# mindspore-lab/mindpose

Hardware: AMD Instinct MI355X
Metric: images/sec at 256x192, HRNet-W32 top-down inference (backbone+head+decode) (higher is better)
Workload: dtype f32; 1 GPU; configs[2]: HRNet-W32 256x192 inference, 1xMI355X per rank, multi-branch conv + fuse layers on fp32 MFMA, HRNetHead, arg-max+shift decode; per_gpu_batch=128, global_batch=128, image=256x192, heatmap=64x48x17, execution_lanes=4

## Files before the change

include/mindpose_hip.h:

```cpp
#ifndef MINDPOSE_HIP_H
#define MINDPOSE_HIP_H

#include <stddef.h>
#include <stdint.h>

#ifdef __cplusplus
extern "C" {
#endif

typedef void* mp_stream_t;

#define MP_OK 0
#define MP_ERR_NULL (-1)
#define MP_ERR_SHAPE (-2)
#define MP_ERR_UNSUPPORTED (-3)
#define MP_ERR_HIP (-4)
#define MP_ERR_WORKSPACE (-5)

const char* mp_version(void);
const char* mp_error_string(int code);
int mp_last_hip_error(void);

#define MP_REFINE_NONE 0
#define MP_REFINE_SHIFT 1
// ... 40 lines not shown

typedef struct mp_conv_desc {
    int32_t n, cin, h, w;
    int32_t cout, kh, kw;
    int32_t stride;
    int32_t pad_top, pad_left;
    int32_t conv_h, conv_w;
    int32_t out_h, out_w;
    int32_t out_mul, out_rep, out_off_y, out_off_x;
    int32_t relu;
    int32_t flags;
} mp_conv_desc;

#define MP_CONV_SHARES_CUS 1
#define MP_CONV_PHASES4 2

size_t mp_conv_packed_weight_bytes(int cout, int cin, int kh, int kw);
int mp_conv_pack_weight(const float* w_dev, float* packed_dev, int cout, int cin, int kh, int kw,
                        int transposed, int phase_y, int phase_x, mp_stream_t stream);
int mp_conv2d_fwd(const mp_conv_desc* desc, const float* x_dev, const float* packed_w_dev,
                  const float* scale_dev, const float* shift_dev, const float* res1_dev, const float* res2_dev,
                  float* out_dev, mp_stream_t stream);

int mp_conv2d_fwd_variant(const mp_conv_desc* desc, int variant, const float* x_dev, const float* packed_w_dev,
                          const float* scale_dev, const float* shift_dev, const float* res1_dev, const float* res2_dev,
                          float* out_dev, mp_stream_t stream);

size_t mp_conv_winograd_packed_weight_bytes(int cout, int cin);
int mp_conv_winograd_pack_weight(const float* w_dev, float* packed_dev, int cout, int cin, mp_stream_t stream);
int mp_conv_winograd_supported(const mp_conv_desc* desc);
int mp_conv2d_winograd_fwd(const mp_conv_desc* desc, const float* x_dev, const float* packed_u_dev, const float* scale_dev,
                           const float* shift_dev, const float* res1_dev, const float* res2_dev, float* out_dev,
                           mp_stream_t stream);

int mp_maxpool3x3s2_same(const float* x_dev, float* out_dev, int n, int c, int h, int w, mp_stream_t stream);

int mp_fuse_upsample_sum(const float* base_dev, const float* t1_dev, int s1, const float* t2_dev, int s2,
                         const float* t3_dev, int s3, float* out_dev, int n, int c, int h, int w, int relu,
                         mp_stream_t stream);

typedef struct mp_plan mp_plan;
mp_plan* mp_plan_create(void);
void mp_plan_destroy(mp_plan* plan);
int mp_plan_add_conv(mp_plan* plan, const mp_conv_desc* desc, const float* x_dev, const float* packed_w_dev,
                     const float* scale_dev, const float* shift_dev, const float* res1_dev,
                     const float* res2_dev, float* out_dev);
int mp_plan_add_conv_variant(mp_plan* plan, const mp_conv_desc* desc, int variant, const float* x_dev,
                             const float* packed_w_dev, const float* scale_dev, const float* shift_dev,
                             const float* res1_dev, const float* res2_dev, float* out_dev);
int mp_deconv4x4s2_gemm_supported(const mp_conv_desc* phase00_desc);
int mp_deconv4x4s2_gemm_fwd(const mp_conv_desc* phase00_desc, const float* x_dev, const float* packed4_dev, const float* scale_dev,
                            const float* shift_dev, float* out_dev, mp_stream_t stream);
int mp_plan_add_deconv4x4s2_gemm(mp_plan* plan, const mp_conv_desc* phase00_desc, const float* x_dev, const float* packed4_dev,
                                 const float* scale_dev, const float* shift_dev, float* out_dev);
int mp_plan_add_conv_winograd(mp_plan* plan, const mp_conv_desc* desc, const float* x_dev, const float* packed_u_dev,
                              const float* scale_dev, const float* shift_dev, const float* res1_dev, const float* res2_dev,
                              float* out_dev);
int mp_plan_add_maxpool(mp_plan* plan, const float* x_dev, float* out_dev, int n, int c, int h, int w);
int mp_plan_add_fuse_sum(mp_plan* plan, const float* base_dev, const float* t1_dev, int s1, const float* t2_dev, int s2,
                         const float* t3_dev, int s3, float* out_dev, int n, int c, int h, int w, int relu);
int mp_plan_set_lane(mp_plan* plan, int lane);
int mp_plan_add_barrier(mp_plan* plan);
int mp_plan_size(const mp_plan* plan);
int mp_plan_run(const mp_plan* plan, mp_stream_t stream);
int mp_plan_run_range(const mp_plan* plan, int first, int count, mp_stream_t stream);
int mp_plan_entry_info(const mp_plan* plan, int index, int64_t info[12]);

size_t mp_bn_workspace_bytes(int c);
int mp_bn_train_fwd(const float* z_dev, const float* gamma_dev, const float* beta_dev, const float* res_dev, float* y_dev,
                    float* save_mean_dev, float* save_invstd_dev, float* moving_mean_dev, float* moving_var_dev, int n,
                    int c, int hw, float eps, float momentum, int relu, void* workspace_dev, size_t workspace_bytes,
                    mp_stream_t stream);
int mp_bn_train_bwd(const float* dy_dev, const float* z_dev, const float* y_dev, const float* gamma_dev,
                    const float* save_mean_dev, const float* save_invstd_dev, float* dz_dev, float* dres_dev,
                    float* dgamma_dev, float* dbeta_dev, int n, int c, int hw, int relu, void* workspace_dev,
                    size_t workspace_bytes, mp_stream_t stream);

int mp_fuse_upsample_sum_bwd(const float* dy_dev, const float* out_dev, float* dbase_dev, float* dt1_dev, int s1,
                             float* dt2_dev, int s2, float* dt3_dev, int s3, int n, int c, int h, int w, int relu,
                             mp_stream_t stream);

int mp_bn_train_bwd_acc(const float* dy_dev, const float* z_dev, const float* y_dev, const float* gamma_dev,
                        const float* save_mean_dev, const float* save_invstd_dev, float* dz_dev, float* dres_dev,
                        float* dgamma_dev, float* dbeta_dev, float* dgamma_acc_dev, float* dbeta_acc_dev, int n, int c, int hw,
                        int relu, void* workspace_dev, size_t workspace_bytes, mp_stream_t stream);

int mp_adamw_step(float* param_dev, const float* grad_dev, float* exp_avg_dev, float* exp_avg_sq_dev, size_t count,
                  float lr, float beta1, float beta2, float eps, float weight_decay, mp_stream_t stream);

int mp_adamw_step_scaled(float* param_dev, const float* grad_dev, float* exp_avg_dev, float* exp_avg_sq_dev, size_t count,
// ... 338 lines not shown
```

mindpose_amd/_lib.py:

```python
import ctypes
import os

import torch

_HERE = os.path.dirname(os.path.abspath(__file__))
LIB_PATH = os.environ.get("MINDPOSE_HIP_LIB", os.path.join(_HERE, "csrc", "libmindpose_hip.so"))

MP_REFINE_NONE, MP_REFINE_SHIFT, MP_REFINE_DARK = 0, 1, 2
MP_CONV_SHARES_CUS = 1
MP_CONV_PHASES4 = 2
MP_ERR_UNSUPPORTED = -3


def env_on(name: str, default: bool = True) -> bool:
    value = os.environ.get(name)
    return value != "0" if default else value == "1"


c_f32p = ctypes.c_void_p
c_int = ctypes.c_int
c_size_t = ctypes.c_size_t
c_i64 = ctypes.c_longlong


# ... 31 lines not shown

class BnBwdJob(ctypes.Structure):
    _fields_ = [(k, ctypes.c_void_p) for k in ("g", "z", "gamma", "save_mean", "save_invstd", "dz", "dgamma", "dbeta", "dgamma_acc",
                                                "dbeta_acc", "partials", "workspace")] + [("workspace_bytes", ctypes.c_size_t)] + \
               [(k, ctypes.c_int) for k in ("n", "c", "hw", "n_parts")]


_PROTOTYPES = {
    "mp_version": (ctypes.c_char_p, []),
    "mp_error_string": (ctypes.c_char_p, [c_int]),
    "mp_last_hip_error": (c_int, []),
    "mp_decode_topdown": (c_int, [c_f32p] * 7 + [c_int] * 7 + [ctypes.c_float, c_f32p, c_int, ctypes.c_void_p]),
    "mp_decode_topdown_debug": (c_int, [c_f32p] * 7 + [c_int] * 7 + [ctypes.c_float, c_f32p, c_int, c_f32p, ctypes.c_void_p]),
    "mp_flip_aggregate": (c_int, [c_f32p] * 4 + [c_int] * 5 + [ctypes.c_void_p]),
    "mp_flip_aggregate_decode": (c_int, [c_f32p] * 3 + [c_int] + [c_f32p] * 7 + [c_int] * 7
                                 + [ctypes.c_float, c_f32p, c_int, ctypes.c_void_p]),
    "mp_gaussian_target": (c_int, [c_f32p, c_f32p, c_int, c_f32p, c_f32p, c_f32p] + [c_int] * 4
                           + [ctypes.c_double] * 3 + [c_int, ctypes.c_void_p]),
    "mp_joints_mse_workspace_bytes": (c_size_t, [c_int, c_int]),
    "mp_joints_mse_fwd": (c_int, [c_f32p] * 5 + [c_size_t] + [c_int] * 3 + [ctypes.c_void_p]),
    "mp_joints_mse_bwd": (c_int, [c_f32p] * 5 + [c_int] * 3 + [ctypes.c_void_p]),
    "mp_joints_ohkm_workspace_bytes": (c_size_t, [c_int, c_int]),
    "mp_joints_ohkm_fwd": (c_int, [c_f32p] * 7 + [c_size_t] + [c_int] * 4 + [ctypes.c_void_p]),
    "mp_joints_ohkm_bwd": (c_int, [c_f32p] * 6 + [c_int] * 4 + [ctypes.c_void_p]),
    "mp_conv_packed_weight_bytes": (c_size_t, [c_int] * 4),
    "mp_conv_pack_weight": (c_int, [c_f32p, c_f32p] + [c_int] * 7 + [ctypes.c_void_p]),
    "mp_conv2d_fwd": (c_int, [ctypes.POINTER(ConvDesc)] + [c_f32p] * 7 + [ctypes.c_void_p]),
    "mp_conv2d_fwd_variant": (c_int, [ctypes.POINTER(ConvDesc), c_int] + [c_f32p] * 7 + [ctypes.c_void_p]),
    "mp_conv_winograd_packed_weight_bytes": (c_size_t, [c_int] * 2),
    "mp_conv_winograd_pack_weight": (c_int, [c_f32p, c_f32p, c_int, c_int, ctypes.c_void_p]),
    "mp_conv_winograd_supported": (c_int, [ctypes.POINTER(ConvDesc)]),
    "mp_conv2d_winograd_fwd": (c_int, [ctypes.POINTER(ConvDesc)] + [c_f32p] * 7 + [ctypes.c_void_p]),
    "mp_plan_add_conv_winograd": (c_int, [ctypes.c_void_p, ctypes.POINTER(ConvDesc)] + [c_f32p] * 7),
    "mp_plan_add_conv_variant": (c_int, [ctypes.c_void_p, ctypes.POINTER(ConvDesc), c_int] + [c_f32p] * 7),
    "mp_deconv4x4s2_gemm_supported": (c_int, [ctypes.POINTER(ConvDesc)]),
    "mp_deconv4x4s2_gemm_fwd": (c_int, [ctypes.POINTER(ConvDesc)] + [c_f32p] * 5 + [ctypes.c_void_p]),
    "mp_plan_add_deconv4x4s2_gemm": (c_int, [ctypes.c_void_p, ctypes.POINTER(ConvDesc)] + [c_f32p] * 5),
    "mp_maxpool3x3s2_same": (c_int, [c_f32p, c_f32p] + [c_int] * 4 + [ctypes.c_void_p]),
    "mp_fuse_upsample_sum": (c_int, [c_f32p, c_f32p, c_int, c_f32p, c_int, c_f32p, c_int, c_f32p] + [c_int] * 5 + [ctypes.c_void_p]),
    "mp_plan_add_fuse_sum": (c_int, [ctypes.c_void_p, c_f32p, c_f32p, c_int, c_f32p, c_int, c_f32p, c_int, c_f32p] + [c_int] * 5),
    "mp_plan_create": (ctypes.c_void_p, []),
    "mp_plan_destroy": (None, [ctypes.c_void_p]),
    "mp_plan_add_conv": (c_int, [ctypes.c_void_p, ctypes.POINTER(ConvDesc)] + [c_f32p] * 7),
    "mp_plan_add_maxpool": (c_int, [ctypes.c_void_p, c_f32p, c_f32p] + [c_int] * 4),
    "mp_plan_size": (c_int, [ctypes.c_void_p]),
    "mp_plan_run": (c_int, [ctypes.c_void_p, ctypes.c_void_p]),
    "mp_plan_run_range": (c_int, [ctypes.c_void_p, c_int, c_int, ctypes.c_void_p]),
    "mp_plan_entry_info": (c_int, [ctypes.c_void_p, c_int, ctypes.POINTER(ctypes.c_int64)]),
    "mp_debug_set_stamp_buffer": (c_int, [ctypes.c_void_p, c_size_t]),
    "mp_bn_workspace_bytes": (c_size_t, [c_int]),
    "mp_bn_train_fwd": (c_int, [c_f32p] * 9 + [c_int] * 3 + [ctypes.c_float, ctypes.c_float, c_int, c_f32p, c_size_t, ctypes.c_void_p]),
    "mp_bn_train_bwd": (c_int, [c_f32p] * 10 + [c_int] * 4 + [c_f32p, c_size_t, ctypes.c_void_p]),
    "mp_bn_train_bwd_acc": (c_int, [c_f32p] * 12 + [c_int] * 4 + [c_f32p, c_size_t, ctypes.c_void_p]),
    "mp_fuse_upsample_sum_bwd": (c_int, [c_f32p, c_f32p, c_f32p, c_f32p, c_int, c_f32p, c_int, c_f32p, c_int] + [c_int] * 5 + [ctypes.c_void_p]),
    "mp_conv_wgrad_workspace_bytes": (c_size_t, [ctypes.POINTER(ConvDesc)]),
    "mp_conv_wgrad": (c_int, [ctypes.POINTER(ConvDesc), c_f32p, c_f32p, c_f32p, c_int, c_f32p, c_size_t, ctypes.c_void_p]),
    "mp_adamw_step": (c_int, [c_f32p] * 4 + [c_size_t] + [ctypes.c_float] * 5 + [ctypes.c_void_p]),
    "mp_adamw_step_scaled": (c_int, [c_f32p] * 4 + [c_size_t] + [ctypes.c_float] * 6 + [c_f32p, ctypes.c_void_p]),
    "mp_grad_finite_check": (c_int, [c_f32p, c_size_t, c_f32p, ctypes.c_void_p]),
    "mp_comm_available": (c_int, []),
    "mp_comm_last_error": (c_int, []),
    "mp_comm_get_unique_id": (c_int, [ctypes.c_void_p]),
    "mp_comm_init_rank": (c_int, [ctypes.POINTER(ctypes.c_void_p), c_int, ctypes.c_void_p, c_int]),
    "mp_comm_destroy": (c_int, [ctypes.c_void_p]),
    "mp_comm_count": (c_int, [ctypes.c_void_p]),
    "mp_allreduce_grads": (c_int, [ctypes.c_void_p, c_f32p, c_size_t, c_int, ctypes.c_void_p]),
# ... 175 lines not shown
```

mindpose_amd/csrc/common.h:

```cpp
#pragma once
#include <hip/hip_runtime.h>
#include <stdint.h>
#include <stdlib.h>

#include <initializer_list>

#include "../../include/mindpose_hip.h"

namespace mp {

extern thread_local int g_last_hip_error;
extern thread_local bool g_dry_launch;

inline int check_launch() {
    hipError_t e = hipGetLastError();
    if (e != hipSuccess) {
        g_last_hip_error = (int)e;
        return MP_ERR_HIP;
    }
    return MP_OK;
}

inline hipStream_t as_stream(mp_stream_t s) { return reinterpret_cast<hipStream_t>(s); }

// ... 15 lines not shown
    if (once.need()) {
        (void)hipFuncSetAttribute(reinterpret_cast<const void*>(Kern), hipFuncAttributeMaxDynamicSharedMemorySize, 160 * 1024);
        (void)hipGetLastError();
    }
    hipLaunchKernelGGL(Kern, grid, block, lds_bytes, s, args...);
    return check_launch();
}

__device__ __forceinline__ int xcd_contiguous(int b, int nb) {
    const int q8 = nb >> 3, r8 = nb & 7, xcd = b & 7, j = b >> 3;
    return (xcd < r8 ? xcd * (q8 + 1) : r8 * (q8 + 1) + (xcd - r8) * q8) + j;
}

constexpr unsigned kOob = 0x80000000u;
__device__ __forceinline__ __amdgpu_buffer_rsrc_t make_rsrc(const void* base, size_t bytes) {
    return __builtin_amdgcn_make_buffer_rsrc(const_cast<void*>(base), 0, (int)(bytes < 0x7FFFFFF0u ? bytes : 0x7FFFFFF0u), 0x00020000);
}

inline unsigned magic_of(unsigned d) { return d <= 1 ? 0u : (unsigned)(0x100000000ULL / d) + 1u; }
__device__ __forceinline__ unsigned fastdiv(unsigned e, unsigned d, unsigned magic) { return d == 1 ? e : __umulhi(e, magic); }

inline int round_up(int v, int m) { return (v + m - 1) / m * m; }

inline bool knobs_on() {
    static const bool on = [] {
        const char* e = getenv("MINDPOSE_EXPERIMENT_KNOBS");
        return e != nullptr && atoi(e) != 0;
    }();
    return on;
}
inline const char* knob(const char* name) { return knobs_on() ? getenv(name) : nullptr; }

enum PlanKind { kConv = 0, kMaxPool = 1, kFuseSum = 2, kConvF16 = 3, kFuseSumF16 = 4, kToC8 = 5, kFromC8 = 6, kBarrier = 7, kBlockF16 = 8,
                kWinograd = 9, kPwChainF16 = 10, kStemF16 = 11, kStemF32 = 12, kPwChainF32 = 13, kConcat = 14, kColSlice = 15 };

inline void fill_info(int64_t info[12], std::initializer_list<int64_t> values) {
    int i = 0;
    for (int64_t v : values) info[i++] = v;
    for (; i < 12; ++i) info[i] = 0;
}

}
```

mindpose_amd/csrc/conv_api.hip:

```cpp
#include <stdlib.h>
#include <string.h>

#include <type_traits>
#include <variant>
#include <vector>

#include "conv_f16.h"
#include "conv_mfma.h"
#include "conv_pw.h"
#include "conv_wino.h"
#include "conv_stem.h"
#include "conv_gemm.h"
#include "conv_small.h"
#include "pwchain_f32.h"

namespace mp {

__device__ __forceinline__ float pack_source(const float* __restrict__ w, int cout, int cin, int kh, int kw, int transposed,
                                             int py, int px, int co, int ci, int t) {
    const int ty = t / kw, tx = t % kw;
    if (transposed == 0) return w[(((size_t)co * cin + ci) * kh + ty) * kw + tx];
    if (transposed == 2) {
        return w[(((size_t)ci * cout + co) * kh + (kh - 1 - ty)) * kw + (kw - 1 - tx)];
    }
    if (transposed == 3) {
        const int ky = py == 0 ? (ty == 0 ? 1 : -1) : (ty == 0 ? 2 : 0);
        const int kx = px == 0 ? (tx == 0 ? 1 : -1) : (tx == 0 ? 2 : 0);
        return (ky < 0 || kx < 0) ? 0.f : w[(((size_t)ci * cout + co) * 3 + ky) * 3 + kx];
    }
    if (transposed == 4) {
        const int my = 1 - ty, mx = 1 - tx;
        const int ky = py == 0 ? 3 - 2 * my : 2 - 2 * my;
        const int kx = px == 0 ? 3 - 2 * mx : 2 - 2 * mx;
        return w[(((size_t)co * cin + ci) * 4 + ky) * 4 + kx];
    }
    const int ky = py == 0 ? 3 - 2 * ty : 2 - 2 * ty;
    const int kx = px == 0 ? 3 - 2 * tx : 2 - 2 * tx;
    return w[(((size_t)ci * cout + co) * 4 + ky) * 4 + kx];
}

__global__ __launch_bounds__(256) void pack_weight_kernel(const float* __restrict__ w, float* __restrict__ out, int cout,
                                                          int cin, int kh, int kw, int cin_pad4, int cout_pad16,
                                                          int transposed, int py, int px) {
    const int T = kh * kw;
// ... 83 lines not shown
                     variant_light(L.variant) ? 1 : 0});
}

struct MaxPool { const float* x; float* out; int n, c, h, w; };
struct FuseSum { const float* base; const float* t[3]; int s[3]; float* out; int n, c, h, w, relu; };
struct FuseSumF16 { const void* base; const void* t[3]; int s[3]; void* out; int n, c, h, w, relu; };
struct ToC8 { const float* x; void* out; int n, c, h, w; };
struct FromC8 { const void* x; float* out; int n, c, h, w; };
struct Concat { const void* a; int ca; const void* b; int cb; void* out; int n, h, w, c8; };
struct ColSlice { const void* in; void* out; int rows, w_in, start, w_out, c8; };
struct Barrier {};

static int run(const MaxPool& r, hipStream_t s) { return mp_maxpool3x3s2_same(r.x, r.out, r.n, r.c, r.h, r.w, s); }
static int run(const FuseSum& r, hipStream_t s) {
    return mp_fuse_upsample_sum(r.base, r.t[0], r.s[0], r.t[1], r.s[1], r.t[2], r.s[2], r.out, r.n, r.c, r.h, r.w, r.relu, s);
}
static int run(const FuseSumF16& r, hipStream_t s) {
    return mp_f16_fuse_upsample_sum(r.base, r.t[0], r.s[0], r.t[1], r.s[1], r.t[2], r.s[2], r.out, r.n, r.c, r.h, r.w, r.relu, s);
}
static int run(const ToC8& r, hipStream_t s) { return mp_f16_to_c8(r.x, r.out, r.n, r.c, r.h, r.w, s); }
static int run(const FromC8& r, hipStream_t s) { return mp_f16_from_c8(r.x, r.out, r.n, r.c, r.h, r.w, s); }
static int run(const Concat& r, hipStream_t s) { return mp_concat_channels(r.a, r.ca, r.b, r.cb, r.out, r.n, r.h, r.w, r.c8, s); }
static int run(const ColSlice& r, hipStream_t s) { return mp_col_slice(r.in, r.out, r.rows, r.w_in, r.start, r.w_out, r.c8, s); }
static int run(const Barrier&, hipStream_t) { return MP_OK; }
static void describe(const MaxPool&, int64_t info[12]) { fill_info(info, {kMaxPool}); }
static void describe(const FuseSum&, int64_t info[12]) { fill_info(info, {kFuseSum}); }
static void describe(const FuseSumF16&, int64_t info[12]) { fill_info(info, {kFuseSumF16}); }
static void describe(const ToC8&, int64_t info[12]) { fill_info(info, {kToC8}); }
static void describe(const FromC8&, int64_t info[12]) { fill_info(info, {kFromC8}); }
static void describe(const Concat&, int64_t info[12]) { fill_info(info, {kConcat}); }
static void describe(const ColSlice&, int64_t info[12]) { fill_info(info, {kColSlice}); }
static void describe(const Barrier&, int64_t info[12]) { fill_info(info, {kBarrier}); }

using Record = std::variant<DirectLaunch, PwLaunch, GemmLaunch, SmallLaunch, WinoLaunch, StemF32Launch, PwChainF32Launch, ConvF16Launch,
                            BlockF16Launch, PwChainLaunch, StemF16Launch, MaxPool, FuseSum, FuseSumF16, ToC8, FromC8, Concat, ColSlice, Barrier>;
template <typename R>
constexpr bool is_f32_conv = std::is_same_v<R, DirectLaunch> || std::is_same_v<R, PwLaunch> || std::is_same_v<R, GemmLaunch> || std::is_same_v<R, SmallLaunch>;

static int run_record(const Record& rec, hipStream_t s) {
    return std::visit([s](const auto& r) { return run(r, s); }, rec);
}

static const int kLdsMax = 150 * 1024;

static int lds_budget() {
    static int v = -1;
    if (v < 0) {
        const char* e = knob("MP_CONV_LDS_KB");
        int kb = e ? atoi(e) : 0;
        v = (kb >= 16 && kb <= 150) ? kb * 1024 : 78 * 1024;
    }
    return v;
}

static int plane_pad(int raw) {
    int v = (raw + 15) / 32 * 32 + 16;
    if (v - 32 >= raw) v -= 32;
    return v;
}

static bool configure(const mp_conv_desc& d, int variant, DirectLaunch& L) {
    int CT, PT;
    variant_dims(variant, CT, PT);
    if (d.kh == 7 && variant != V_CT64_PT192 && variant != V_CT32_PT192_H) return false;
    ConvKParams& p = L.p;
    const int S = d.stride, KS = d.kh;
    p.N = d.n; p.Cin = d.cin; p.H = d.h; p.W = d.w; p.Cout = d.cout;
// ... 340 lines not shown

int mp_plan_add_maxpool(mp_plan* plan, const float* x, float* out, int n, int c, int h, int w) {
    if (!plan || !x || !out) return MP_ERR_NULL;
    if (n <= 0 || c <= 0 || h <= 0 || w <= 0) return MP_ERR_SHAPE;
    return push(plan, MaxPool{x, out, n, c, h, w});
}

int mp_plan_add_fuse_sum(mp_plan* plan, const float* base, const float* t1, int s1, const float* t2, int s2,
                         const float* t3, int s3, float* out, int n, int c, int h, int w, int relu) {
    if (!plan || !base || !t1 || !out) return MP_ERR_NULL;
    if (n <= 0 || c <= 0 || h <= 0 || w <= 0) return MP_ERR_SHAPE;
    return push(plan, FuseSum{base, {t1, t2, t3}, {s1, s2, s3}, out, n, c, h, w, relu});
}

int mp_plan_add_conv_f16(mp_plan* plan, const mp_conv_desc* desc, int variant, const void* x, const void* packed_w,
                         const float* scale, const float* shift, const void* res1, const void* res2, void* out) {
    if (!plan) return MP_ERR_NULL;
    ConvF16Launch L{};
    int rc = f16_build_launch(desc, variant, x, packed_w, scale, shift, res1, res2, out, L);
    return rc != MP_OK ? rc : push(plan, L);
}

int mp_plan_add_conv_winograd(mp_plan* plan, const mp_conv_desc* desc, const float* x, const float* packed_u, const float* scale,
                              const float* shift, const float* res1, const float* res2, float* out) {
    if (!plan) return MP_ERR_NULL;
    WinoLaunch L{};
    int rc = wino_configure(desc, L);
    if (rc != MP_OK) return rc;
    if (!x || !packed_u || !scale || !shift || !out) return MP_ERR_NULL;
    L.p.x = x; L.p.u = packed_u; L.p.scale = scale; L.p.shift = shift; L.p.res1 = res1; L.p.res2 = res2; L.p.out = out;
    return push(plan, L);
}

int mp_plan_add_basicblock_f16(mp_plan* plan, const void* x, const void* packed_w1, const float* scale1, const float* shift1,
                               const void* packed_w2, const float* scale2, const float* shift2, void* out, int n, int c, int h,
                               int w, int rows) {
    if (!plan) return MP_ERR_NULL;
    BlockF16Launch L{};
    int rc = blockf16_build(x, packed_w1, scale1, shift1, packed_w2, scale2, shift2, out, n, c, h, w, rows, L);
    return rc != MP_OK ? rc : push(plan, L);
}

int mp_plan_add_expand_reduce_f16(mp_plan* plan, const void* mid, const void* res, const void* packed_w3, const float* scale3,
                                  const float* shift3, int relu3, const void* packed_w1, const float* scale1, const float* shift1,
                                  int relu1, void* y, void* z, int n, int cm, int ce, int cr, int h, int w) {
    if (!plan) return MP_ERR_NULL;
    PwChainLaunch L{};
    int rc = pwchain_build(mid, res, packed_w3, scale3, shift3, relu3, packed_w1, scale1, shift1, relu1, y, z, n, cm, ce, cr, h, w, L);
    return rc != MP_OK ? rc : push(plan, L);
}

int mp_plan_add_expand_reduce(mp_plan* plan, const float* mid, const float* res, const float* x0, const float* packed_wd, const float* scale_d,
                              const float* shift_d, const float* packed_w3, const float* scale3, const float* shift3, const float* packed_w1,
                              const float* scale1, const float* shift1, float* y, float* z, int n, int cm, int ce, int cr, int h, int w) {
    if (!plan) return MP_ERR_NULL;
    PwChainF32Launch L{};
    int rc = pwchain32_build(mid, res, x0, packed_wd, scale_d, shift_d, packed_w3, scale3, shift3, packed_w1, scale1, shift1, y, z, n, cm, ce, cr,
                             h, w, L);
    return rc != MP_OK ? rc : push(plan, L);
}

int mp_plan_add_ds_expand_reduce_f16(mp_plan* plan, const void* mid, const void* x0, const void* packed_wd, const float* scale_d,
                                     const float* shift_d, const void* packed_w3, const float* scale3, const float* shift3, int relu3,
                                     const void* packed_w1, const float* scale1, const float* shift1, int relu1, void* y, void* z, int n,
                                     int cm, int ce, int cr, int h, int w) {
    if (!plan || !x0) return MP_ERR_NULL;
// ... 101 lines not shown
```

mindpose_amd/models/backbones/hrnet.py:

```python
import contextlib
import os
from typing import Dict, List, Tuple, Type, Union

import torch
import torch.nn as nn

from ...register import register
from .. import train_ops as T
from ..layers import BatchNorm2d, Conv2d, Plan
from .backbone import Backbone
from .utils import load_pretrained

__all__ = ["HRNet", "hrnet_w32", "hrnet_w48"]


class BasicBlock(nn.Module):

    expansion: int = 1

    def __init__(self, in_channels: int, channels: int, stride: int = 1, down_sample: nn.Module = None) -> None:
        super().__init__()
        self.conv1 = Conv2d(in_channels, channels, 3, stride=stride, padding=1)
        self.bn1 = BatchNorm2d(channels)
        self.conv2 = Conv2d(channels, channels, 3, stride=1, padding=1)
# ... 352 lines not shown
                chain = []
                for j in range(i + 1 - len(pre)):
                    cout = cur[i] if j == i - len(pre) else pre[-1]
                    chain.append(_conv_bn(pre[-1], cout, 3, stride=2, padding=1, relu=True))
                layers.append(nn.Sequential(*chain))
                flags.append(True)
        return nn.ModuleList(layers), flags

    def _make_layer(self, block, in_channels: int, out_channels: int, blocks: int, stride: int = 1) -> nn.Sequential:
        down = None
        if stride != 1 or in_channels != out_channels * block.expansion:
            down = _conv_bn(in_channels, out_channels * block.expansion, 1, stride=stride)
        layers = [block(in_channels, out_channels, stride, down_sample=down)]
        for _ in range(1, blocks):
            layers.append(block(out_channels * block.expansion, out_channels))
        return nn.Sequential(*layers)

    def _make_stage(self, cfg, num_inchannels, multi_scale_output: bool = True):
        block = self.blocks_dict[cfg["block"]]
        modules = []
        for i in range(cfg["num_modules"]):
            mso = not (not multi_scale_output and i == cfg["num_modules"] - 1)
            modules.append(HRModule(cfg["num_branches"], block, cfg["num_blocks"], num_inchannels,
                                    cfg["num_channels"], mso))
            num_inchannels = modules[-1].num_inchannels
        return nn.Sequential(*modules), num_inchannels

    def emit(self, plan: Plan, x: torch.Tensor) -> torch.Tensor:
        if plan.fuses_stem(x, self.conv1):
            x = plan.stem(x, self.conv1, self.bn1)
        else:
            x = plan.enter(x)
            x = plan.conv(x, self.conv1, self.bn1, relu=True)
        x = plan.conv(x, self.conv2, self.bn2, relu=True)
        x = emit_block_sequence(plan, list(self.layer1), x)
        ys = [x]
        for idx in (2, 3, 4):
            trans = getattr(self, f"transition{idx - 1}")
            flags = getattr(self, f"transition{idx - 1}_flags")
            cfg = getattr(self, f"stage{idx}_cfg")
            xs = []
            for i in range(cfg["num_branches"]):
                plan.set_lane(min(i, len(ys) - 1))
                if not flags[i]:
                    xs.append(ys[i])
                elif i < len(ys):
                    xs.append(_emit_conv_bn(plan, trans[i], ys[i]))
                else:
                    t = ys[-1]
                    for seq in trans[i]:
                        t = _emit_conv_bn(plan, seq, t)
                    xs.append(t)
            plan.barrier()
            for mod in getattr(self, f"stage{idx}"):
                xs = mod.emit(plan, xs)
            ys = xs
        plan.set_lane(0)
        return ys[0]

    def train_forward(self, x: torch.Tensor) -> torch.Tensor:
        if self.amp_level in ("O2", "O3") and not T._is_c8(x):
            x = T.to_c8(x)
        x = T.conv_bn_act(x, self.conv1, self.bn1, relu=True)
        x = T.conv_bn_act(x, self.conv2, self.bn2, relu=True)
        for blk in self.layer1:
            x = blk.train_forward(x)
        if x.requires_grad and x.is_cuda:
            x.register_hook(_flush_queued_weight_gradients)
        ys = [x]
        cuts = getattr(self, "_train_cut_sink", None)
        cut_at = getattr(self, "_train_cut_at", None)
        for idx in (2, 3, 4):
            if cuts is not None and (cut_at is None or idx - 2 in cut_at):
                leaves = []
                for y in ys:
                    leaf = y.detach().requires_grad_()
                    link = getattr(y, "_mp_bn_link", None)
                    if link is not None:
                        leaf._mp_bn_link = link
                    leaves.append(leaf)
                cuts.append((list(ys), leaves))
                ys = leaves
            trans = getattr(self, f"transition{idx - 1}")
            flags = getattr(self, f"transition{idx - 1}_flags")
# ... 57 lines not shown
```

mindpose_amd/models/layers.py:

```python
import ctypes
from typing import Dict, List, Optional, Tuple

import torch
import torch.nn as nn

from .. import _lib
from .act_c8 import ActC8
from .tuner import (BLOCK_ROWS, F16_VARIANTS, F32_SMALL_WIDE, F32_WINOGRAD, _autotune, autotune_on, tune_conv_variant, tuned,
                    winograd_enabled)
from .tuner import _TUNE_MIN_MACS

BN_EPS = 1e-5


class Conv2d(nn.Module):

    def __init__(self, in_channels: int, out_channels: int, kernel_size: int, stride: int = 1, padding: int = 0,
                 has_bias: bool = False) -> None:
        super().__init__()
        self.in_channels, self.out_channels = in_channels, out_channels
        self.kernel_size, self.stride, self.padding = kernel_size, stride, padding
        self.weight = nn.Parameter(torch.empty(out_channels, in_channels, kernel_size, kernel_size))
        self.bias = nn.Parameter(torch.zeros(out_channels)) if has_bias else None

# ... 232 lines not shown

    def _pack_winograd(self, weight: torch.Tensor, cout: int, cin: int) -> torch.Tensor:
        key = (id(weight), "wino")
        if key in self._packed:
            return self._packed[key]
        w = weight.detach().to(self.device, torch.float32).contiguous()
        packed = torch.empty(self.lib.mp_conv_winograd_packed_weight_bytes(cout, cin) // 4, device=self.device, dtype=torch.float32)
        _lib.check(self.lib.mp_conv_winograd_pack_weight(_lib.ptr(w), _lib.ptr(packed), cout, cin, _lib.stream()),
                   "mp_conv_winograd_pack_weight")
        self.keep += [w, packed]
        self._packed[key] = packed
        return packed

    def _affine(self, cout: int, bn: Optional[BatchNorm2d], bias: Optional[torch.Tensor], half: bool = False):
        key = (id(bn) if bn is not None else None, id(bias) if bias is not None else None, cout, half)
        if key in self._folded:
            return self._folded[key]
        if bn is not None:
            scale, shift = bn.folded()
            scale, shift = scale.to(self.device), shift.to(self.device)
        else:
            scale = torch.ones(cout, device=self.device)
            shift = bias.detach().float().to(self.device).contiguous() if bias is not None else torch.zeros(cout, device=self.device)
        if half:
            pad = (-cout) % 16
            scale = torch.cat([scale, scale.new_zeros(pad)]).contiguous()
            shift = torch.cat([shift, shift.new_zeros(pad)]).contiguous()
        self.keep += [scale, shift]
        self._folded[key] = (scale, shift)
        return scale, shift

    def conv(self, x: torch.Tensor, conv: Conv2d, bn: Optional[BatchNorm2d] = None, relu: bool = False,
             res1: Optional[torch.Tensor] = None, res2: Optional[torch.Tensor] = None,
             out: Optional[torch.Tensor] = None, upsample: int = 1) -> torch.Tensor:
        n, cin, h, w = x.shape
        k, s, pad, cout = conv.kernel_size, conv.stride, conv.padding, conv.out_channels
        if cin != conv.in_channels:
            raise ValueError(f"conv expects {conv.in_channels} input channels, got {cin}")
        half = isinstance(x, ActC8)
        if half and upsample != 1:
            raise NotImplementedError("fp16 plans add up-sampled terms with fuse_sum, not through the conv epilogue")
        ho = (h + 2 * pad - k) // s + 1
        wo = (w + 2 * pad - k) // s + 1
        d = conv_desc(n, cin, h, w, cout, k, s, pad, pad, ho, wo, ho * upsample, wo * upsample, upsample, upsample, relu=relu)
        if upsample == 1 and not self._conv_served(d, half, int(res1 is not None) + int(res2 is not None)):
            return self._conv_by_columns(x, conv, bn, relu, res1, res2, out)
        out = self._conv_out(x, d, res1, res2, out)
        return self._record_conv(d, x, self._pack(conv.weight, cout, cin, k, False, 0, 0, half), *self._affine(cout, bn, conv.bias, half),
                                 res1, res2, out, "conv_f16" if half else "conv", packed_u=self._winograd_weight(d, conv, half))

    def _conv_out(self, x, d, res1, res2, out):
        shape = (d.n, d.cout, d.out_h, d.out_w)
        if out is None:
            out = self._alloc_like(x, *shape)
        if tuple(out.shape) != shape:
            raise ValueError(f"bad out shape {tuple(out.shape)}")
        for r in (res1, res2):
            if r is not None and tuple(r.shape) != shape:
                raise ValueError(f"residual shape {tuple(r.shape)} != out shape {shape}")
        return out

    def _winograd_weight(self, d, conv: Conv2d, half: bool):
        if half or not (winograd_enabled() and autotune_on()) or self.lib.mp_conv_winograd_supported(ctypes.byref(d)) != 0:
            return None
        return self._pack_winograd(conv.weight, conv.out_channels, conv.in_channels)

    def _record_conv(self, d, x, packed, scale, shift, res1, res2, out, kind: str, packed_u=None, variant: Optional[int] = None):
        half = isinstance(x, ActC8)
        if variant is None:
            variant = tune_conv_variant(self.lib, d, x, packed, scale, shift, res1, res2, out, half=half, packed_u=packed_u)
        operands = [_lib.ptr(t) for t in (scale, shift, res1, res2, out)]
        if not half and variant == F32_WINOGRAD:
            kind = "conv_winograd"
            _lib.check(self.lib.mp_plan_add_conv_winograd(self.handle, ctypes.byref(d), _lib.ptr(x), _lib.ptr(packed_u), *operands),
                       "mp_plan_add_conv_winograd")
        else:
            add = self.lib.mp_plan_add_conv_f16 if half else self.lib.mp_plan_add_conv_variant
            _lib.check(add(self.handle, ctypes.byref(d), variant, _lib.ptr(x), _lib.ptr(packed), *operands), f"mp_plan_add_conv ({kind})")
        self._conv_info(kind, d.kh, d.stride, d.cin, d.cout, d.h, d.w, d.n, _macs(d))
        return out

    def _conv_served(self, d, half: bool, n_res: int) -> bool:
        picks = tuned(_macs(d))
        if half:
            return any(self.lib.mp_f16_conv_supported(ctypes.byref(d), v, n_res, 0) == 1 for v in range(-1, F16_VARIANTS if picks else 0))
        if any(self.lib.mp_conv_supported(ctypes.byref(d), v) == 1 for v in range(-1, F32_SMALL_WIDE + 1 if picks else 0)):
            return True
        return picks and winograd_enabled() and self.lib.mp_conv_winograd_supported(ctypes.byref(d)) == 0

    def _fewest_bands(self, bands_of, half: bool, n_res: int, what: str):
        for nb in range(2, 33):
            bands = bands_of(nb)
            if all(self._conv_served(d, half, n_res) for _, _, d in bands):
                return bands
        raise _lib.MindposeHipError(f"no kernel serves the {what}, not even in column bands")

    def col_slice(self, x, start: int, width: int):
        n, c, h, w = x.shape
        half = isinstance(x, ActC8)
        out = self._alloc_like(x, n, c, h, width)
        rows = n * ((c + 7) // 8 if half else c) * h
        _lib.check(self.lib.mp_plan_add_col_slice(self.handle, _lib.ptr(x), _lib.ptr(out), rows, w, start, width, int(half)),
                   "mp_plan_add_col_slice")
        self.layer_info.append(dict(kind="col_slice", n=n, c=c, h=h, w=width, macs=0))
        return out

    def _conv_by_columns(self, x, conv: Conv2d, bn, relu, res1, res2, out):
        n, cin, h, w = x.shape
        k, s, pad, cout = conv.kernel_size, conv.stride, conv.padding, conv.out_channels
        half = isinstance(x, ActC8)
        bands = self._fewest_bands(lambda nb: conv_column_bands(n, cin, h, w, cout, k, s, pad, relu, nb), half,
                                   int(res1 is not None) + int(res2 is not None),
# ... 344 lines not shown
```

Before: 9658 images/s.

## Add streaming fp32 MFMA kernel for stride-2 3x3 convs with 64 outputs

Adds a dedicated kernel for 3x3 stride-2 convolutions with 64 output channels. It streams input channels in chunks of 8 through LDS, prefetches the next chunk in registers while MFMA runs on the current one, and stores even and odd columns as deinterleaved halves so the strided taps read contiguously. It is wired into the stem conv2 and the stage-2 transition convs, and autotuning chooses between it and the existing variant, which falls back safely. The cost is a second packed weight copy, more autotune work at plan build, and extra code to maintain.

```diff
diff --git a/include/mindpose_hip.h b/include/mindpose_hip.h
--- a/include/mindpose_hip.h
+++ b/include/mindpose_hip.h
@@ -96,6 +96,12 @@
 int mp_conv2d_winograd_fwd(const mp_conv_desc* desc, const float* x_dev, const float* packed_u_dev, const float* scale_dev,
                            const float* shift_dev, const float* res1_dev, const float* res2_dev, float* out_dev,
                            mp_stream_t stream);
+
+size_t mp_conv_s2stream_packed_weight_bytes(int cin);
+int mp_conv_s2stream_pack_weight(const float* w_dev, float* packed_dev, int cin, mp_stream_t stream);
+int mp_conv_s2stream_supported(const mp_conv_desc* desc);
+int mp_conv2d_s2stream_fwd(const mp_conv_desc* desc, const float* x_dev, const float* packed_w_dev, const float* scale_dev,
+                           const float* shift_dev, float* out_dev, mp_stream_t stream);
 
 int mp_maxpool3x3s2_same(const float* x_dev, float* out_dev, int n, int c, int h, int w, mp_stream_t stream);
 
@@ -120,6 +126,8 @@
 int mp_plan_add_conv_winograd(mp_plan* plan, const mp_conv_desc* desc, const float* x_dev, const float* packed_u_dev,
                               const float* scale_dev, const float* shift_dev, const float* res1_dev, const float* res2_dev,
                               float* out_dev);
+int mp_plan_add_conv_s2stream(mp_plan* plan, const mp_conv_desc* desc, const float* x_dev, const float* packed_w_dev,
+                              const float* scale_dev, const float* shift_dev, float* out_dev);
 int mp_plan_add_maxpool(mp_plan* plan, const float* x_dev, float* out_dev, int n, int c, int h, int w);
 int mp_plan_add_fuse_sum(mp_plan* plan, const float* base_dev, const float* t1_dev, int s1, const float* t2_dev, int s2,
                          const float* t3_dev, int s3, float* out_dev, int n, int c, int h, int w, int relu);
diff --git a/mindpose_amd/_lib.py b/mindpose_amd/_lib.py
--- a/mindpose_amd/_lib.py
+++ b/mindpose_amd/_lib.py
@@ -87,6 +87,11 @@
     "mp_conv_winograd_supported": (c_int, [ctypes.POINTER(ConvDesc)]),
     "mp_conv2d_winograd_fwd": (c_int, [ctypes.POINTER(ConvDesc)] + [c_f32p] * 7 + [ctypes.c_void_p]),
     "mp_plan_add_conv_winograd": (c_int, [ctypes.c_void_p, ctypes.POINTER(ConvDesc)] + [c_f32p] * 7),
+    "mp_conv_s2stream_packed_weight_bytes": (c_size_t, [c_int]),
+    "mp_conv_s2stream_pack_weight": (c_int, [c_f32p, c_f32p, c_int, ctypes.c_void_p]),
+    "mp_conv_s2stream_supported": (c_int, [ctypes.POINTER(ConvDesc)]),
+    "mp_conv2d_s2stream_fwd": (c_int, [ctypes.POINTER(ConvDesc)] + [c_f32p] * 5 + [ctypes.c_void_p]),
+    "mp_plan_add_conv_s2stream": (c_int, [ctypes.c_void_p, ctypes.POINTER(ConvDesc)] + [c_f32p] * 5),
     "mp_plan_add_conv_variant": (c_int, [ctypes.c_void_p, ctypes.POINTER(ConvDesc), c_int] + [c_f32p] * 7),
     "mp_deconv4x4s2_gemm_supported": (c_int, [ctypes.POINTER(ConvDesc)]),
     "mp_deconv4x4s2_gemm_fwd": (c_int, [ctypes.POINTER(ConvDesc)] + [c_f32p] * 5 + [ctypes.c_void_p]),
diff --git a/mindpose_amd/csrc/common.h b/mindpose_amd/csrc/common.h
--- a/mindpose_amd/csrc/common.h
+++ b/mindpose_amd/csrc/common.h
@@ -71,7 +71,7 @@
 inline const char* knob(const char* name) { return knobs_on() ? getenv(name) : nullptr; }
 
 enum PlanKind { kConv = 0, kMaxPool = 1, kFuseSum = 2, kConvF16 = 3, kFuseSumF16 = 4, kToC8 = 5, kFromC8 = 6, kBarrier = 7, kBlockF16 = 8,
-                kWinograd = 9, kPwChainF16 = 10, kStemF16 = 11, kStemF32 = 12, kPwChainF32 = 13, kConcat = 14, kColSlice = 15 };
+                kWinograd = 9, kPwChainF16 = 10, kStemF16 = 11, kStemF32 = 12, kPwChainF32 = 13, kConcat = 14, kColSlice = 15, kConvS2Stream = 16 };
 
 inline void fill_info(int64_t info[12], std::initializer_list<int64_t> values) {
     int i = 0;
diff --git a/mindpose_amd/csrc/conv_api.hip b/mindpose_amd/csrc/conv_api.hip
--- a/mindpose_amd/csrc/conv_api.hip
+++ b/mindpose_amd/csrc/conv_api.hip
@@ -10,6 +10,7 @@
 #include "conv_pw.h"
 #include "conv_wino.h"
 #include "conv_stem.h"
+#include "conv_s2_stream.h"
 #include "conv_gemm.h"
 #include "conv_small.h"
 #include "pwchain_f32.h"
@@ -159,7 +160,7 @@
 static void describe(const ColSlice&, int64_t info[12]) { fill_info(info, {kColSlice}); }
 static void describe(const Barrier&, int64_t info[12]) { fill_info(info, {kBarrier}); }
 
-using Record = std::variant<DirectLaunch, PwLaunch, GemmLaunch, SmallLaunch, WinoLaunch, StemF32Launch, PwChainF32Launch, ConvF16Launch,
+using Record = std::variant<DirectLaunch, PwLaunch, GemmLaunch, SmallLaunch, WinoLaunch, StemF32Launch, S2StreamLaunch, PwChainF32Launch, ConvF16Launch,
                             BlockF16Launch, PwChainLaunch, StemF16Launch, MaxPool, FuseSum, FuseSumF16, ToC8, FromC8, Concat, ColSlice, Barrier>;
 template <typename R>
 constexpr bool is_f32_conv = std::is_same_v<R, DirectLaunch> || std::is_same_v<R, PwLaunch> || std::is_same_v<R, GemmLaunch> || std::is_same_v<R, SmallLaunch>;
@@ -566,6 +567,17 @@
     return push(plan, L);
 }
 
+int mp_plan_add_conv_s2stream(mp_plan* plan, const mp_conv_desc* desc, const float* x, const float* packed_w, const float* scale,
+                              const float* shift, float* out) {
+    if (!plan) return MP_ERR_NULL;
+    S2StreamLaunch L{};
+    int rc = s2stream_configure(desc, L);
+    if (rc != MP_OK) return rc;
+    if (!x || !packed_w || !scale || !shift || !out) return MP_ERR_NULL;
+    L.p.x = x; L.p.wp = packed_w; L.p.scale = scale; L.p.shift = shift; L.p.out = out;
+    return push(plan, L);
+}
+
 int mp_plan_add_basicblock_f16(mp_plan* plan, const void* x, const void* packed_w1, const float* scale1, const float* shift1,
                                const void* packed_w2, const float* scale2, const float* shift2, void* out, int n, int c, int h,
                                int w, int rows) {
diff --git a/mindpose_amd/csrc/conv_s2_stream.h b/mindpose_amd/csrc/conv_s2_stream.h
--- /dev/null
+++ b/mindpose_amd/csrc/conv_s2_stream.h
@@ -0,0 +1,38 @@
+#pragma once
+#include "common.h"
+
+namespace mp {
+
+struct S2StreamParams {
+    const float* x;
+    const float* wp;
+    const float* scale;
+    const float* shift;
+    float* out;
+    int N, Cin, H, W, Ho, Wo;
+    int R, RIN;
+    int RP, CP, half;
+    int n_chunks, tiles_y, total_blocks, band_px, units, upr, relu;
+    unsigned magic_upr, magic_rin, magic_wo;
+    unsigned long long* dbg;
+};
+struct S2StreamLaunch {
+    S2StreamParams p;
+    size_t lds_bytes;
+};
+
+constexpr int kS2Chunk = 8;
+constexpr int kS2Tiles = 12;
+constexpr int kS2WChunk = kS2Chunk * 9 * 64;
+
+int s2stream_configure(const mp_conv_desc* d, S2StreamLaunch& L);
+int s2stream_launch(const S2StreamLaunch& L, hipStream_t s);
+int s2stream_pack_launch(const float* w, float* packed, int cin, hipStream_t s);
+unsigned long long* conv_stamp_buffer(size_t need_bytes);
+
+inline int run(const S2StreamLaunch& L, hipStream_t s) { return s2stream_launch(L, s); }
+inline void describe(const S2StreamLaunch& L, int64_t info[12]) {
+    fill_info(info, {kConvS2Stream, 3, 2, 0, L.p.total_blocks, (int64_t)L.lds_bytes, 64, L.p.band_px, kS2Chunk, 1, L.p.R});
+}
+
+}
diff --git a/mindpose_amd/csrc/conv_s2_stream_f32.hip b/mindpose_amd/csrc/conv_s2_stream_f32.hip
--- /dev/null
+++ b/mindpose_amd/csrc/conv_s2_stream_f32.hip
@@ -0,0 +1,250 @@
+#include "conv_mfma.h"
+#include "conv_s2_stream.h"
+
+namespace mp {
+
+namespace {
+
+constexpr int kCK = kS2Chunk, kP = kS2Tiles / 4, kNI = 7;
+constexpr int kNW = (kS2WChunk / 4 + 255) / 256;
+
+__global__ __launch_bounds__(256, 2) void conv_s2_stream_f32_kernel(const S2StreamParams p) {
+    extern __shared__ __attribute__((aligned(16))) float lds_s2[];
+    float* lds_w = lds_s2;
+    float* lds_x = lds_s2 + kS2WChunk;
+    const int tid = threadIdx.x, lane = tid & 63;
+    const int wave = __builtin_amdgcn_readfirstlane(tid >> 6);
+    const int lq = lane >> 4, lr = lane & 15;
+    const int CP = p.CP, RP = p.RP, half = p.half;
+    MP_STAMP(t_start);
+    [[maybe_unused]] unsigned long long s_mm = 0, s_st = 0;
+    const int b = xcd_contiguous(blockIdx.x, p.total_blocks);
+    const int n = b / p.tiles_y, y0 = (b - n * p.tiles_y) * p.R;
+
+    int goff[kNI], loff[kNI];
+#pragma unroll
+    for (int i = 0; i < kNI; ++i) {
+        const unsigned u = (unsigned)(tid + 256 * i);
+        const int cr = (int)fastdiv(u, (unsigned)p.upr, p.magic_upr), xu = (int)u - cr * p.upr;
+        const int c = (int)fastdiv((unsigned)cr, (unsigned)p.RIN, p.magic_rin), r = cr - c * p.RIN;
+        const int yin = 2 * y0 - 1 + r;
+        const bool ok = (int)u < p.units;
+        loff[i] = ok ? c * CP + r * RP + 2 * xu : -1;
+        goff[i] = ok && yin >= 0 && yin < p.H ? (c * p.H + yin) * p.W + 4 * xu : -1;
+    }
+    int abase[kP];
+#pragma unroll
+    for (int i = 0; i < kP; ++i) {
+        int pp = 16 * (wave * kP + i) + lr;
+        pp = pp < p.band_px ? pp : p.band_px - 1;
+        const int ry = (int)fastdiv((unsigned)pp, (unsigned)p.Wo, p.magic_wo), ox = pp - ry * p.Wo;
+        abase[i] = lq * CP + 2 * ry * RP + ox;
+    }
+    float sc[4], sh[4];
+#pragma unroll
+    for (int cb = 0; cb < 4; ++cb) {
+        sc[cb] = p.scale[16 * cb + lr];
+        sh[cb] = p.shift[16 * cb + lr];
+    }
+    const float* img = p.x + (size_t)n * p.Cin * p.H * p.W;
+    const size_t chunk_stride = (size_t)kCK * p.H * p.W;
+
+    float4 xv[kNI], wv[kNW];
+    auto fetch = [&](int chunk) {
+        const float* xc = img + chunk * chunk_stride;
+#pragma unroll
+        for (int i = 0; i < kNI; ++i) {
+            xv[i] = make_float4(0.f, 0.f, 0.f, 0.f);
+            if (goff[i] >= 0) xv[i] = *reinterpret_cast<const float4*>(xc + goff[i]);
+        }
+        const float4* wc = reinterpret_cast<const float4*>(p.wp + (size_t)chunk * kS2WChunk);
+#pragma unroll
+        for (int j = 0; j < kNW; ++j) {
+            wv[j] = make_float4(0.f, 0.f, 0.f, 0.f);
+            if (256 * j + tid < kS2WChunk / 4) wv[j] = wc[256 * j + tid];
+        }
+    };
+    auto stage = [&]() {
+#pragma unroll
+        for (int i = 0; i < kNI; ++i)
+            if (loff[i] >= 0) {
+                float* d = lds_x + loff[i];
+                d[0] = xv[i].x; d[half + 1] = xv[i].y; d[1] = xv[i].z; d[half + 2] = xv[i].w;
+            }
+#pragma unroll
+        for (int j = 0; j < kNW; ++j)
+            if (256 * j + tid < kS2WChunk / 4) reinterpret_cast<float4*>(lds_w)[256 * j + tid] = wv[j];
+    };
+
+    fetch(0);
+    for (int i = tid; i < kCK * p.RIN; i += 256) {
+        const int c = (int)fastdiv((unsigned)i, (unsigned)p.RIN, p.magic_rin);
+        lds_x[c * CP + (i - c * p.RIN) * RP + half] = 0.f;
+    }
+    stage();
+    __syncthreads();
+    MP_STAMP(t_pro);
+
+    f32x4 acc[kP][4];
+#pragma unroll
+    for (int i = 0; i < kP; ++i)
+#pragma unroll
+        for (int cb = 0; cb < 4; ++cb) acc[i][cb] = (f32x4){0.f, 0.f, 0.f, 0.f};
+
+    for (int chunk = 0; chunk < p.n_chunks; ++chunk) {
+        MP_STAMP(t0);
+        const bool more = chunk + 1 < p.n_chunks;
+        if (more) fetch(chunk + 1);
+        f32x4 bw[2];
+        float a[2][kP];
+        auto read_step = [&](int s, int slot) {
+            const int tap = s >> 1, g = s & 1, ky = tap / 3, kx = tap - 3 * ky;
+            const int xoff = ky * RP + (kx == 1 ? 0 : half + (kx >> 1)) + 4 * g * CP;
+            bw[slot] = *reinterpret_cast<const f32x4*>(lds_w + (s * 64 + lane) * 4);
+#pragma unroll
+            for (int i = 0; i < kP; ++i) a[slot][i] = lds_x[abase[i] + xoff];
+        };
+        read_step(0, 0);
+#pragma unroll
+        for (int s = 0; s < 18; ++s) {
+            if (s + 1 < 18) read_step(s + 1, (s + 1) & 1);
+            __builtin_amdgcn_sched_barrier(0);
+#pragma unroll
+            for (int i = 0; i < kP; ++i)
+#pragma unroll
+                for (int cb = 0; cb < 4; ++cb)
+                    acc[i][cb] = __builtin_amdgcn_mfma_f32_16x16x4f32(a[s & 1][i], bw[s & 1][cb], acc[i][cb], 0, 0, 0);
+            __builtin_amdgcn_sched_barrier(0);
+        }
+        MP_STAMP(t1);
+        __syncthreads();
+        if (more) stage();
+        __syncthreads();
+        MP_STAMP(t2);
+        s_mm += t1 - t0;
+        s_st += t2 - t1;
+    }
+
+    const size_t plane_o = (size_t)p.Ho * p.Wo;
+    float* outn = p.out + (size_t)n * 64 * plane_o + (size_t)y0 * p.Wo;
+    const int px_left = (p.Ho - y0) * p.Wo;
+#pragma unroll
+    for (int i = 0; i < kP; ++i) {
+        const int p4 = 16 * (wave * kP + i) + 4 * lq;
+        if (p4 < p.band_px && p4 < px_left) {
+#pragma unroll
+            for (int cb = 0; cb < 4; ++cb) {
+                f32x4 v = acc[i][cb] * sc[cb] + sh[cb];
+                if (p.relu) { v.x = fmaxf(v.x, 0.f); v.y = fmaxf(v.y, 0.f); v.z = fmaxf(v.z, 0.f); v.w = fmaxf(v.w, 0.f); }
+                *reinterpret_cast<f32x4*>(outn + (size_t)(16 * cb + lr) * plane_o + p4) = v;
+            }
+        }
+    }
+#if MP_CONV_STAMPS
+    {
+        MP_STAMP(t_end);
+        if (p.dbg && tid == 0) {
+            unsigned long long* d = p.dbg + (size_t)blockIdx.x * 8;
+            d[0] = t_start; d[1] = t_pro - t_start; d[2] = s_mm; d[3] = s_st; d[4] = t_end;
+            d[5] = 0; d[6] = 0; d[7] = 0;
+        }
+    }
+#endif
+}
+
+__global__ __launch_bounds__(256) void pack_weight_s2_stream_kernel(const float* __restrict__ w, float* __restrict__ out, int cin) {
+    const int total = cin / kCK * kS2WChunk;
+    for (int i = blockIdx.x * blockDim.x + threadIdx.x; i < total; i += gridDim.x * blockDim.x) {
+        const int cb = i & 3, lane = (i >> 2) & 63, kg = (i >> 8) % 18, chunk = i / kS2WChunk;
+        const int co = 16 * cb + (lane & 15), ci = kCK * chunk + 4 * (kg & 1) + (lane >> 4), tap = kg >> 1;
+        out[i] = w[((size_t)co * cin + ci) * 9 + tap];
+    }
+}
+
+}
+
+int s2stream_pack_launch(const float* w, float* packed, int cin, hipStream_t s) {
+    if (!w || !packed) return MP_ERR_NULL;
+    if (cin <= 0) return MP_ERR_SHAPE;
+    if (cin % kCK) return MP_ERR_UNSUPPORTED;
+    const int blocks = (cin / kCK * kS2WChunk + 255) / 256;
+    hipLaunchKernelGGL(pack_weight_s2_stream_kernel, dim3(blocks < 1024 ? blocks : 1024), dim3(256), 0, s, w, packed, cin);
+    return check_launch();
+}
+
+int s2stream_configure(const mp_conv_desc* d, S2StreamLaunch& L) {
+    if (!d) return MP_ERR_NULL;
+    if (d->n <= 0 || d->cin <= 0 || d->cout <= 0 || d->h <= 0 || d->w <= 0) return MP_ERR_SHAPE;
+    if (d->kh != 3 || d->kw != 3 || d->stride != 2 || d->pad_top != 1 || d->pad_left != 1) return MP_ERR_UNSUPPORTED;
+    if (d->cout != 64 || (d->cin % kCK) || (d->h & 1) || (d->w & 15)) return MP_ERR_UNSUPPORTED;
+    if (d->w > 192) return MP_ERR_UNSUPPORTED;
+    if (d->conv_h != d->h / 2 || d->conv_w != d->w / 2 || d->out_h != d->conv_h || d->out_w != d->conv_w) return MP_ERR_UNSUPPORTED;
+    if (d->out_mul != 1 || d->out_rep != 1 || d->out_off_y != 0 || d->out_off_x != 0) return MP_ERR_UNSUPPORTED;
+    if (d->flags & ~MP_CONV_SHARES_CUS) return MP_ERR_UNSUPPORTED;
+    if ((long long)d->cin * d->h * d->w >= 0x1FFFFFF0LL) return MP_ERR_UNSUPPORTED;
+    S2StreamParams& p = L.p;
+    p.N = d->n; p.Cin = d->cin; p.H = d->h; p.W = d->w; p.Ho = d->h / 2; p.Wo = d->w / 2; p.relu = d->relu ? 1 : 0;
+    p.half = p.Wo;
+    p.upr = p.W / 4;
+    int r = kS2Tiles * 16 / p.Wo;
+    if (r > p.Ho) r = p.Ho;
+    while (r > 1 && kCK * (2 * r + 1) * p.upr > kNI * 256) --r;
+    if (r < 1 || kCK * (2 * r + 1) * p.upr > kNI * 256) return MP_ERR_UNSUPPORTED;
+    if (const char* e = knob("MP_CONV_S2_ROWS")) {
+        const int v = atoi(e);
+        if (v >= 1 && v < r) r = v;
+    }
+    p.R = r; p.RIN = 2 * r + 1;
+    p.band_px = r * p.Wo;
+    p.units = kCK * p.RIN * p.upr;
+    p.RP = p.W + 1;
+    while ((2 * p.RP - p.Wo) & 31) ++p.RP;
+    p.CP = (p.RIN * p.RP + 15) / 32 * 32 + 16;
+    if (p.CP - 32 >= p.RIN * p.RP) p.CP -= 32;
+    p.n_chunks = p.Cin / kCK;
+    p.tiles_y = (p.Ho + r - 1) / r;
+    if ((long long)p.N * p.tiles_y >= 0x7FFFFFFFLL) return MP_ERR_UNSUPPORTED;
+    p.total_blocks = p.N * p.tiles_y;
+    p.magic_upr = magic_of((unsigned)p.upr);
+    p.magic_rin = magic_of((unsigned)p.RIN);
+    p.magic_wo = magic_of((unsigned)p.Wo);
+    L.lds_bytes = (size_t)(kS2WChunk + kCK * p.CP) * 4;
+    if (L.lds_bytes > 150 * 1024) return MP_ERR_UNSUPPORTED;
+    return MP_OK;
+}
+
+int s2stream_launch(const S2StreamLaunch& L0, hipStream_t s) {
+    if (g_dry_launch) return MP_OK;
+    S2StreamLaunch L = L0;
+    L.p.dbg = conv_stamp_buffer((size_t)L.p.total_blocks * 64);
+    return launch_lds<conv_s2_stream_f32_kernel>(dim3(L.p.total_blocks), dim3(256), L.lds_bytes, s, L.p);
+}
+
+}
+
+using namespace mp;
+
+extern "C" {
+
+size_t mp_conv_s2stream_packed_weight_bytes(int cin) { return cin > 0 && cin % kS2Chunk == 0 ? (size_t)cin / kS2Chunk * kS2WChunk * sizeof(float) : 0; }
+
+int mp_conv_s2stream_pack_weight(const float* w, float* packed, int cin, mp_stream_t stream) {
+    return s2stream_pack_launch(w, packed, cin, as_stream(stream));
+}
+
+int mp_conv_s2stream_supported(const mp_conv_desc* desc) {
+    S2StreamLaunch L{};
+    return s2stream_configure(desc, L);
+}
+
+int mp_conv2d_s2stream_fwd(const mp_conv_desc* desc, const float* x, const float* packed_w, const float* scale, const float* shift,
+                           float* out, mp_stream_t stream) {
+    S2StreamLaunch L{};
+    int rc = s2stream_configure(desc, L);
+    if (rc != MP_OK) return rc;
+    if (!x || !packed_w || !scale || !shift || !out) return MP_ERR_NULL;
+    L.p.x = x; L.p.wp = packed_w; L.p.scale = scale; L.p.shift = shift; L.p.out = out;
+    return s2stream_launch(L, as_stream(stream));
+}
+
+}
diff --git a/mindpose_amd/models/backbones/hrnet.py b/mindpose_amd/models/backbones/hrnet.py
--- a/mindpose_amd/models/backbones/hrnet.py
+++ b/mindpose_amd/models/backbones/hrnet.py
@@ -408,7 +408,7 @@
         else:
             x = plan.enter(x)
             x = plan.conv(x, self.conv1, self.bn1, relu=True)
-        x = plan.conv(x, self.conv2, self.bn2, relu=True)
+        x = plan.conv(x, self.conv2, self.bn2, relu=True, s2stream=True)
         x = emit_block_sequence(plan, list(self.layer1), x)
         ys = [x]
         for idx in (2, 3, 4):
@@ -425,7 +425,7 @@
                 else:
                     t = ys[-1]
                     for seq in trans[i]:
-                        t = _emit_conv_bn(plan, seq, t)
+                        t = _emit_conv_bn(plan, seq, t, s2stream=idx == 2)
                     xs.append(t)
             plan.barrier()
             for mod in getattr(self, f"stage{idx}"):
diff --git a/mindpose_amd/models/layers.py b/mindpose_amd/models/layers.py
--- a/mindpose_amd/models/layers.py
+++ b/mindpose_amd/models/layers.py
@@ -288,7 +288,7 @@
 
     def conv(self, x: torch.Tensor, conv: Conv2d, bn: Optional[BatchNorm2d] = None, relu: bool = False,
              res1: Optional[torch.Tensor] = None, res2: Optional[torch.Tensor] = None,
-             out: Optional[torch.Tensor] = None, upsample: int = 1) -> torch.Tensor:
+             out: Optional[torch.Tensor] = None, upsample: int = 1, s2stream: bool = False) -> torch.Tensor:
         n, cin, h, w = x.shape
         k, s, pad, cout = conv.kernel_size, conv.stride, conv.padding, conv.out_channels
         if cin != conv.in_channels:
@@ -302,6 +302,8 @@
         if upsample == 1 and not self._conv_served(d, half, int(res1 is not None) + int(res2 is not None)):
             return self._conv_by_columns(x, conv, bn, relu, res1, res2, out)
         out = self._conv_out(x, d, res1, res2, out)
+        if s2stream and upsample == 1 and res1 is None and res2 is None and self.fuses_s2stream(x, conv, d):
+            return self._conv_s2stream(d, x, conv, bn, out)
         return self._record_conv(d, x, self._pack(conv.weight, cout, cin, k, False, 0, 0, half), *self._affine(cout, bn, conv.bias, half),
                                  res1, res2, out, "conv_f16" if half else "conv", packed_u=self._winograd_weight(d, conv, half))
 
@@ -334,6 +336,41 @@
             add = self.lib.mp_plan_add_conv_f16 if half else self.lib.mp_plan_add_conv_variant
             _lib.check(add(self.handle, ctypes.byref(d), variant, _lib.ptr(x), _lib.ptr(packed), *operands), f"mp_plan_add_conv ({kind})")
         self._conv_info(kind, d.kh, d.stride, d.cin, d.cout, d.h, d.w, d.n, _macs(d))
+        return out
+
+    def fuses_s2stream(self, x: torch.Tensor, conv: Conv2d, d) -> bool:
+        if isinstance(x, ActC8) or conv.bias is not None or not _lib.env_on("MINDPOSE_CONV_S2STREAM"):
+            return False
+        return self.lib.mp_conv_s2stream_supported(ctypes.byref(d)) == 0
+
+    def _conv_s2stream(self, d, x, conv: Conv2d, bn, out):
+        cin, cout = conv.in_channels, conv.out_channels
+        scale, shift = self._affine(cout, bn, None, False)
+        packed = self._pack(conv.weight, cout, cin, 3, False, 0, 0, False)
+        key = (id(conv.weight), "s2stream")
+        if key not in self._packed:
+            w = conv.weight.detach().to(self.device, torch.float32).contiguous()
+            buf = torch.empty(self.lib.mp_conv_s2stream_packed_weight_bytes(cin) // 4, device=self.device, dtype=torch.float32)
+            _lib.check(self.lib.mp_conv_s2stream_pack_weight(_lib.ptr(w), _lib.ptr(buf), cin, _lib.stream()), "mp_conv_s2stream_pack_weight")
+            self.keep += [w, buf]
+            self._packed[key] = buf
+        packed_s = self._packed[key]
+        variant = tune_conv_variant(self.lib, d, x, packed, scale, shift, None, None, out)
+        stream = _lib.stream()
+
+        def launch(form):
+            if form == 1:
+                return self.lib.mp_conv2d_s2stream_fwd(ctypes.byref(d), _lib.ptr(x), _lib.ptr(packed_s), _lib.ptr(scale), _lib.ptr(shift),
+                                                       _lib.ptr(out), stream)
+            return self.lib.mp_conv2d_fwd_variant(ctypes.byref(d), variant, _lib.ptr(x), _lib.ptr(packed), _lib.ptr(scale), _lib.ptr(shift),
+                                                  None, None, _lib.ptr(out), stream)
+
+        tkey = ("conv_s2stream",) + tuple(getattr(d, f) for f, _ in d._fields_) + (str(out.device),)
+        if _autotune(tkey, _macs(d), 2, launch) == 0:
+            return self._record_conv(d, x, packed, scale, shift, None, None, out, "conv", variant=variant)
+        _lib.check(self.lib.mp_plan_add_conv_s2stream(self.handle, ctypes.byref(d), _lib.ptr(x), _lib.ptr(packed_s), _lib.ptr(scale),
+                                                      _lib.ptr(shift), _lib.ptr(out)), "mp_plan_add_conv_s2stream")
+        self._conv_info("conv_s2stream", 3, 2, cin, cout, d.h, d.w, d.n, _macs(d))
         return out
 
     def _conv_served(self, d, half: bool, n_res: int) -> bool:
```

Result: no change. 9680 images/s, median of 6 (+0.2%).
